# swasik/vector-store-text

Measured on AMD Instinct MI355X. Metric: kNN QPS @ recall@10>=0.95 (HNSW, 1000000 x 768 f32 cos), higher is better.
Workload: dtype f32

## Files before the change

### vector-store-text_amd/csrc/hnsw_regset.hpp

```cpp
#pragma once
#include <type_traits>

#include "hnsw_common.hpp"

namespace vsg {

#define VSG_KEY_EMPTY (~0ull)

#ifndef VSG_COMPACT_EARLY
#define VSG_COMPACT_EARLY 0
#endif

__device__ __forceinline__ uint64_t cand_key(float d, uint32_t id) {
    uint32_t b = __float_as_uint(d);
    if (b == 0x80000000u) b = 0u;
    const uint32_t u = (b & 0x80000000u) ? ~b : (b | 0x80000000u);
    return ((uint64_t)u << 32) | (id & VSG_ID_MASK);
}
__device__ __forceinline__ float key_dist(uint64_t k) {
    const uint32_t u = (uint32_t)(k >> 32);
    return __uint_as_float((u & 0x80000000u) ? (u & 0x7FFFFFFFu) : ~u);
}

__device__ __forceinline__ uint64_t shfl_xor64(uint64_t v, int o) {
    const uint32_t lo = (uint32_t)__shfl_xor((int)(uint32_t)v, o);
    const uint32_t hi = (uint32_t)__shfl_xor((int)(uint32_t)(v >> 32), o);
    return ((uint64_t)hi << 32) | lo;
}
__device__ __forceinline__ uint64_t readlane64(uint64_t v, int l) {
    const uint32_t lo = (uint32_t)__builtin_amdgcn_readlane((int)(uint32_t)v, l);
    const uint32_t hi = (uint32_t)__builtin_amdgcn_readlane((int)(uint32_t)(v >> 32), l);
    return ((uint64_t)hi << 32) | lo;
}
template <int CTRL> __device__ __forceinline__ uint64_t dpp64(uint64_t v) {
    const uint32_t lo = (uint32_t)__builtin_amdgcn_mov_dpp((int)(uint32_t)v, CTRL, 0xF, 0xF, false);
    const uint32_t hi = (uint32_t)__builtin_amdgcn_mov_dpp((int)(uint32_t)(v >> 32), CTRL, 0xF, 0xF, false);
    return ((uint64_t)hi << 32) | lo;
}
__device__ __forceinline__ uint64_t wave_min64(uint64_t v) {
#if VSG_DPP_REDUCE
    uint64_t w;
    w = dpp64<0xB1>(v);
    v = w < v ? w : v;
    w = dpp64<0x4E>(v);
    v = w < v ? w : v;
    w = dpp64<0x141>(v);
    v = w < v ? w : v;
    w = dpp64<0x140>(v);
    v = w < v ? w : v;
    const uint64_t r0 = readlane64(v, 0), r1 = readlane64(v, 16), r2 = readlane64(v, 32), r3 = readlane64(v, 48);
    const uint64_t a = r0 < r1 ? r0 : r1, b = r2 < r3 ? r2 : r3;
    return a < b ? a : b;
#else
#pragma unroll
    for (int o = 32; o > 0; o >>= 1) {
        const uint64_t w = shfl_xor64(v, o);
        v = w < v ? w : v;
    }
    return v;
#endif
}

template <int R> struct RegSet {
    uint64_t k[R];
    uint32_t expm;
    int size;
    uint64_t tkey;

    __device__ __forceinline__ void init(uint64_t first) {
#pragma unroll
        for (int r = 0; r < R; ++r) k[r] = VSG_KEY_EMPTY;
        if (lane_id() == 0) k[0] = first;
        expm = 0;
        size = 1;
        tkey = VSG_KEY_EMPTY;
    }

    __device__ __forceinline__ uint64_t min_unexpanded() const {
        uint64_t b = VSG_KEY_EMPTY;
#pragma unroll
        for (int r = 0; r < R; ++r)
            if (!((expm >> r) & 1u) && k[r] < b) b = k[r];
        return wave_min64(b);
    }

    __device__ __forceinline__ int count_below(uint64_t x) const {
        int c = 0;
#pragma unroll
        for (int r = 0; r < R; ++r) c += popc64(__ballot(k[r] < x));
        return c;
    }

    __device__ __forceinline__ void mark_expanded(uint64_t x) {
#pragma unroll
        for (int r = 0; r < R; ++r)
            if (k[r] == x) expm |= 1u << r;
    }

    __device__ __forceinline__ bool contains(uint64_t x) const {
        bool h = false;
#pragma unroll
        for (int r = 0; r < R; ++r) h = h || k[r] == x;
        return __ballot(h) != 0;
    }

    __device__ __forceinline__ void compact(int keep, uint32_t excl = 0) {
        uint32_t ph = 0;
        int need = keep;
#if VSG_COMPACT_EARLY
        int rsize = size;
        const int cap = keep + (64 * (R - 1) - keep) / 2;
#endif
#pragma unroll 1
        for (int b = 31; b >= 0; --b) {
            const uint32_t hm = b == 31 ? 0u : (~0u << (b + 1));
            int c = 0;
#pragma unroll
            for (int r = 0; r < R; ++r) {
                const uint32_t hi = (uint32_t)(k[r] >> 32);
                c += popc64(__ballot(k[r] != VSG_KEY_EMPTY && !((excl >> r) & 1u) && (hi & hm) == ph && !((hi >> b) & 1u)));
            }
            if (c < need) {
                need -= c;
                ph |= 1u << b;
#if VSG_COMPACT_EARLY
                rsize -= c;
#endif
            }
#if VSG_COMPACT_EARLY
            else {
                rsize = c;
            }
            const int kept = keep - need + rsize;
            if (b > 0 && kept <= cap) {
                const uint64_t cut = ((uint64_t)(ph | ((1u << b) - 1u)) << 32) | 0xFFFFFFFFull;
#pragma unroll
                for (int r = 0; r < R; ++r)
                    if (k[r] > cut) {
                        k[r] = VSG_KEY_EMPTY;
                        expm &= ~(1u << r);
                    }
                size = kept;
                tkey = cut;
                return;
            }
#endif
        }
        int ceq = 0;
#pragma unroll
        for (int r = 0; r < R; ++r)
            ceq += popc64(__ballot(k[r] != VSG_KEY_EMPTY && !((excl >> r) & 1u) && (uint32_t)(k[r] >> 32) == ph));
        uint64_t cut;
        if (need == ceq) {
            uint64_t mx = 0;
#pragma unroll
            for (int r = 0; r < R; ++r)
                if (k[r] != VSG_KEY_EMPTY && !((excl >> r) & 1u) && (uint32_t)(k[r] >> 32) == ph && k[r] > mx) mx = k[r];
#pragma unroll
            for (int o = 32; o > 0; o >>= 1) {
                const uint64_t w = shfl_xor64(mx, o);
                mx = w > mx ? w : mx;
            }
            cut = mx;
// ... 23 lines not shown
                expm &= ~(1u << r);
            }
        if (excl) {
            int c = 0;
#pragma unroll
            for (int r = 0; r < R; ++r) c += popc64(__ballot(k[r] != VSG_KEY_EMPTY));
            size = c;
        } else {
            size = keep;
        }
        tkey = cut;
    }

    __device__ __forceinline__ uint64_t bound_ef(int ef) const {
        uint32_t ph = 0;
        int need = ef;
#pragma unroll 1
        for (int b = 31; b >= 16; --b) {
            const uint32_t hm = b == 31 ? 0u : (~0u << (b + 1));
            int c = 0;
#pragma unroll
            for (int r = 0; r < R; ++r) {
                const uint32_t hi = (uint32_t)(k[r] >> 32);
                c += popc64(__ballot(k[r] != VSG_KEY_EMPTY && (hi & hm) == ph && !((hi >> b) & 1u)));
            }
            if (c < need) {
                need -= c;
                ph |= 1u << b;
            }
        }
        return ((uint64_t)(ph | 0xFFFFu) << 32) | 0xFFFFFFFFull;
    }

    __device__ __forceinline__ void fill(const uint64_t* sk, int nc) {
        int acc = 0;
#pragma unroll
        for (int r = 0; r < R; ++r) {
            if (acc < nc) {
                const bool fr = k[r] == VSG_KEY_EMPTY;
                const uint64_t em = __ballot(fr);
                const int idx = acc + lanes_below(em);
                if (fr && idx < nc) {
                    k[r] = sk[idx];
                    expm &= ~(1u << r);
                }
                acc += popc64(em);
            }
        }
        size += nc;
    }
};

template <int R>
__device__ __forceinline__ void admit(RegSet<R>& B, bool mine, uint64_t ck, bool lossy, int ef, uint64_t* sk,
                                      BeamProf* pf = nullptr) {
    (void)pf;
    const int lane = lane_id();
    bool valid = mine && ck < B.tkey;
    uint64_t vm = __ballot(valid);
    if (lossy && vm) {
        for (uint64_t mm = vm; mm; mm &= mm - 1) {
            const int j = __builtin_ctzll(mm);
            if (B.contains(readlane64(ck, j))) vm &= ~(1ull << j);
        }
        valid = (vm >> lane) & 1ull;
    }
    int nc = popc64(vm);
    if (nc && B.size + nc > 64 * R) {
#ifdef VSG_SEARCH_PROFILE
        const uint64_t tc = VSG_CYC();
#endif
        B.compact(ef);
        valid = valid && ck < B.tkey;
        vm = __ballot(valid);
        nc = popc64(vm);
#ifdef VSG_SEARCH_PROFILE
        if (pf) {
            pf->c_comp += VSG_CYC() - tc;
            pf->ncomp++;
        }
#endif
    }
    if (nc) {
        if (valid) sk[lanes_below(vm)] = ck;
        wave_sync();
        B.fill(sk, nc);
        wave_sync();
    }
}

struct NoSketch {};

template <int G, int VM, int U, typename T, int MET, int R, typename PRE = NoSketch>
__device__ __forceinline__ void beam_reg(const GraphDev& g, const QReg<G, VM, T>& q, int l, uint32_t ep, float dep, int ef, WaveLds& w,
                         RegSet<R>& B, uint64_t& ndist, uint64_t& nadj, BeamProf& pf, uint32_t self = VSG_EMPTY,
                         PRE* pre = nullptr) {
    const int lane = lane_id();
    [[maybe_unused]] int tau_size = -1;
    const int m0r = __builtin_amdgcn_readfirstlane(g.M0), mr = __builtin_amdgcn_readfirstlane(g.M);
    const int m = l == 0 ? m0r : mr;
    auto rfl_ptr = [](const uint32_t* p) {
        const uint64_t v = (uint64_t)p;
        const uint32_t lo = (uint32_t)__builtin_amdgcn_readfirstlane((int)(uint32_t)v);
        const uint32_t hi = (uint32_t)__builtin_amdgcn_readfirstlane((int)(uint32_t)(v >> 32));
        return (const uint32_t*)(((uint64_t)hi << 32) | lo);
    };
    const uint32_t* adj0 = rfl_ptr(g.adj0);
    const uint32_t* upper = rfl_ptr(g.upper);
    const uint32_t* upper_off = rfl_ptr(g.upper_off);
    w.vis.clear();
    if (ep != VSG_EMPTY) {
        if (lane == 0) {
            bool unrec;
            w.vis.insert(ep, unrec);
        }
        B.init(cand_key(dep, ep));
    } else {
        wave_sync();
#pragma unroll
        for (int r = 0; r < R; ++r)
            if (B.k[r] != VSG_KEY_EMPTY) {
                bool unrec;
                w.vis.insert((uint32_t)B.k[r] & VSG_ID_MASK, unrec);
            }
        B.expm = 0;
        B.tkey = VSG_KEY_EMPTY;
    }
    bool lossy = false;
    uint64_t* sk = reinterpret_cast<uint64_t*>(w.sd);
    wave_sync();
    auto row_of = [&](uint32_t n) {
        return l == 0 ? adj0 + (size_t)n * m0r : upper + ((size_t)upper_off[n] + (size_t)(l - 1)) * mr;
    };
    for (;;) {
        const uint64_t t0 = VSG_CLK();
        [[maybe_unused]] uint64_t c0c = VSG_CYC();
        const uint64_t a = B.min_unexpanded();
        if (a == VSG_KEY_EMPTY) break;
        if (B.size > ef && B.count_below(a) >= ef) break;
        B.mark_expanded(a);
        const uint32_t na = (uint32_t)a & VSG_ID_MASK;
        const uint32_t* row = row_of(na);
        ++nadj;
#ifdef VSG_SEARCH_PROFILE
        {
            const uint64_t c = VSG_CYC();
            pf.c_sel += c - c0c;
            pf.nexp++;
            c0c = c;
        }
#endif
        for (int c0 = 0; c0 < m; c0 += 64) {
            const uint32_t nb = c0 + lane < m ? row[c0 + lane] : VSG_EMPTY;
            const bool full = __ballot(nb != VSG_EMPTY) == ~0ull;
#ifdef VSG_SEARCH_PROFILE
            {
                const uint64_t c = VSG_CYC();
                pf.c_adj += c - c0c;
                c0c = c;
            }
#endif
            bool fresh = false, evicted = false;
            if (nb != VSG_EMPTY && nb != self) fresh = w.vis.insert(nb, evicted);
            const uint64_t mask = __ballot(fresh);
            lossy = lossy || __ballot(evicted) != 0;
            const int cnt0 = popc64(mask);
            if (fresh) w.todo[lanes_below(mask)] = nb;
            wave_sync();
            const uint64_t t1 = VSG_CLK();
            pf.adj += t1 - t0;
#ifdef VSG_SEARCH_PROFILE
            {
                const uint64_t c = VSG_CYC();
                pf.c_vis += c - c0c;
                c0c = c;
            }
#endif
            int cnt = cnt0;
            if constexpr (!std::is_same<PRE, NoSketch>::value) {
                if (cnt0) {
                    if (B.size >= ef && B.size != tau_size) {
                        const uint64_t tau = B.bound_ef(ef);
                        if (tau < B.tkey) B.tkey = tau;
                        tau_size = B.size;
                    }
                    if (B.tkey != VSG_KEY_EMPTY) cnt = pre->filter(w, cnt0, B.tkey);
                    pre->nexact += (uint32_t)cnt;
                }
            }
            ndist += (uint64_t)cnt0;
            if (cnt) {
#ifdef VSG_SEARCH_PROFILE
                rows_dist<G, VM, U, T, MET>(g.vecs, g.row_bytes, g.nchunks, w.todo, cnt, q, w.tdist, &pf.rows);
#else
                rows_dist<G, VM, U, T, MET>(g.vecs, g.row_bytes, g.nchunks, w.todo, cnt, q, w.tdist);
#endif
                wave_sync();
                const uint64_t ck = lane < cnt ? cand_key(w.tdist[lane], w.todo[lane]) : VSG_KEY_EMPTY;
                const uint64_t t2 = VSG_CLK();
                pf.dist += t2 - t1;
#ifdef VSG_SEARCH_PROFILE
                const uint64_t ca = VSG_CYC();
                admit<R>(B, lane < cnt, ck, lossy, ef, sk, &pf);
                c0c = VSG_CYC();
                pf.c_admit += c0c - ca;
#else
                admit<R>(B, lane < cnt, ck, lossy, ef, sk);
#endif
                pf.merge += VSG_CLK() - t2;
            }
            if (!full) break;
        }
    }
}


struct FiltState {
    uint32_t remm;
    int nlive;
    uint64_t maxlive;
    uint64_t rad0;
    uint32_t overflow;
    bool degraded;
};

__device__ __forceinline__ uint64_t wave_max64(uint64_t v) { return ~wave_min64(~v); }

template <int R> __device__ __forceinline__ int live_below(const RegSet<R>& B, const FiltState& F, uint64_t x) {
    int c = 0;
#pragma unroll
    for (int r = 0; r < R; ++r) c += popc64(__ballot(B.k[r] < x && !((F.remm >> r) & 1u)));
    return c;
}

template <int R> __device__ __forceinline__ void recount(RegSet<R>& B, FiltState& F) {
    int c = 0;
#pragma unroll
    for (int r = 0; r < R; ++r) {
        const bool e = B.k[r] == VSG_KEY_EMPTY;
        if (e) {
            F.remm &= ~(1u << r);
            B.expm &= ~(1u << r);
        }
        c += popc64(__ballot(!e));
    }
    B.size = c;
}

template <int R> __device__ __forceinline__ void compact_filt(RegSet<R>& B, FiltState& F, int ef) {
    if (F.nlive >= ef) {
        B.compact(ef, F.remm);
        F.nlive = ef;
        recount(B, F);
    }
}

template <int R>
__device__ __forceinline__ void fill_filt(RegSet<R>& B, FiltState& F, const uint64_t* sk, const uint32_t* sf, int nc) {
    int acc = 0;
#pragma unroll
    for (int r = 0; r < R; ++r) {
        if (acc < nc) {
            const bool fr = B.k[r] == VSG_KEY_EMPTY;
            const uint64_t em = __ballot(fr);
            const int idx = acc + lanes_below(em);
            if (fr && idx < nc) {
                B.k[r] = sk[idx];
                B.expm &= ~(1u << r);
                if (sf[idx]) F.remm |= 1u << r;
                else F.remm &= ~(1u << r);
            }
            acc += popc64(em);
        }
    }
    B.size += nc;
}

template <int R>
__device__ __forceinline__ void admit_filt(RegSet<R>& B, FiltState& F, bool mine, uint64_t ck, bool rem, bool lossy,
                                           int ef, uint64_t* sk, uint32_t* sf) {
    const int lane = lane_id();
    bool valid = mine && ck < B.tkey && !(F.degraded && rem);
    uint64_t vm = __ballot(valid);
    if (lossy && vm) {
        for (uint64_t mm = vm; mm; mm &= mm - 1) {
            const int j = __builtin_ctzll(mm);
            if (B.contains(readlane64(ck, j))) vm &= ~(1ull << j);
        }
        valid = (vm >> lane) & 1ull;
    }
    int nc = popc64(vm);
    if (nc && B.size + nc > 64 * R) {
        compact_filt(B, F, ef);
        valid = valid && ck < B.tkey;
        vm = __ballot(valid);
        nc = popc64(vm);
        if (B.size + nc > 64 * R) {
            const uint64_t before = (uint64_t)B.size;
#pragma unroll
            for (int r = 0; r < R; ++r)
                if ((F.remm >> r) & 1u) B.k[r] = VSG_KEY_EMPTY;
            recount(B, F);
            F.overflow += (uint32_t)(before - (uint64_t)B.size) + (uint32_t)popc64(__ballot(valid && rem));
            F.degraded = true;
            valid = valid && !rem;
            vm = __ballot(valid);
// ... 143 lines not shown
```

### vector-store-text_amd/csrc/hnsw_search_reg.hip

```cpp
#include <hip/hip_runtime.h>

#include <map>
#include <type_traits>
#include <mutex>
#include <tuple>

#include "hnsw_common.hpp"
#include "hnsw_regset.hpp"
#include "sketch_device.hpp"
#include "vsg_dispatch.hpp"

namespace vsg {

#ifndef VSG_SEARCH_ATTR
#define VSG_SEARCH_ATTR
#endif
template <int G, int VM, int U, typename T, int MET, int R, bool PF>
__device__ __forceinline__ void search_reg_one(const SearchParams& p, int qi, uint8_t* smem) {
    const int lane = lane_id();
    const GraphDev g = to_dev(p.g);
    WaveLds w = carve(smem, 0, p.hash_size, 0);
    uint64_t ndist = 0, nadj = 0;
    BeamProf pf;
    [[maybe_unused]] const uint64_t cq0 = VSG_CYC(), tq0 = VSG_CLK();
    int count = 0;
    uint64_t* ok = p.out_keys + (size_t)qi * p.k;
    float* od = p.out_dist + (size_t)qi * p.k;
    if (p.entry != VSG_EMPTY) {
        QReg<G, VM, T> q;
        q.load(p.queries + (size_t)qi * g.row_bytes, g.nchunks);
        uint32_t cur = p.entry;
        float dcur = dist_one<G, VM, U, T, MET>(g, q, cur, w);
        ++ndist;
        RegSet<R> B;
        using SS = SketchShape<G, VM>;
        using Pre = std::conditional_t<PF, SketchPre<SS::GS, SS::VMS, SS::US>, NoSketch>;
        Pre pre_s;
        Pre* pre = nullptr;
        if constexpr (PF) {
            pre_s.sk = p.sk;
            pre_s.meta = reinterpret_cast<const float2*>(p.sk_meta);
            pre_s.stride = p.sk_stride;
            pre_s.schunks = (int)(p.sk_stride / 16);
            pre_s.q.stage(p.queries + (size_t)qi * g.row_bytes, g.nchunks, p.sk_dim,
                          smem + wave_lds_bytes(p.hash_size, 0, 0));
            pre = &pre_s;
        }
        if (p.upper_ef > 1 && p.max_level >= 1) {
#ifdef VSG_UPPER_ALL_LEVELS
            beam_reg<G, VM, U, T, MET, R>(g, q, p.max_level, cur, dcur, min(p.upper_ef, p.ef), w, B, ndist, nadj, pf);
            for (int l = p.max_level - 1; l >= 1; --l)
                beam_reg<G, VM, U, T, MET, R>(g, q, l, VSG_EMPTY, 0.f, min(p.upper_ef, p.ef), w, B, ndist, nadj, pf);
#else
            for (int l = p.max_level; l >= 2; --l) greedy_level<G, VM, U, T, MET>(g, q, l, cur, dcur, w, ndist, nadj);
            beam_reg<G, VM, U, T, MET, R>(g, q, 1, cur, dcur, min(p.upper_ef, p.ef), w, B, ndist, nadj, pf);
#endif
            beam_reg<G, VM, U, T, MET, R, Pre>(g, q, 0, VSG_EMPTY, 0.f, p.ef, w, B, ndist, nadj, pf, VSG_EMPTY, pre);
        } else {
            [[maybe_unused]] const uint64_t cd0 = VSG_CYC();
            for (int l = p.max_level; l >= 1; --l) greedy_level<G, VM, U, T, MET>(g, q, l, cur, dcur, w, ndist, nadj);
#ifdef VSG_SEARCH_PROFILE
            pf.c_desc += VSG_CYC() - cd0;
#endif
            beam_reg<G, VM, U, T, MET, R, Pre>(g, q, 0, cur, dcur, p.ef, w, B, ndist, nadj, pf, VSG_EMPTY, pre);
        }
        if constexpr (PF) {
            if (lane == 0 && p.stats) {
                atomicAdd(&p.stats[18], (unsigned long long)pre_s.nsketch);
                atomicAdd(&p.stats[19], (unsigned long long)pre_s.nexact);
            }
        }
        uint32_t alive = 0;
#pragma unroll
        for (int r = 0; r < R; ++r)
            if (B.k[r] != VSG_KEY_EMPTY && !(p.flags[(uint32_t)B.k[r] & VSG_ID_MASK] & 1)) alive |= 1u << r;
        uint32_t* sel = w.vis.tab;
        const int lim = min(p.ef, B.size);
        for (int x = 0; x < lim && count < p.k; ++x) {
            uint64_t b = VSG_KEY_EMPTY;
#pragma unroll
            for (int r = 0; r < R; ++r) b = B.k[r] < b ? B.k[r] : b;
            b = wave_min64(b);
            if (b == VSG_KEY_EMPTY) break;
            bool live = false;
#pragma unroll
            for (int r = 0; r < R; ++r)
                if (B.k[r] == b) {
                    live = (alive >> r) & 1u;
                    B.k[r] = VSG_KEY_EMPTY;
                }
            if (__ballot(live)) {
                if (lane == 0) {
                    od[count] = key_dist(b);
                    sel[count] = (uint32_t)b & VSG_ID_MASK;
                }
                ++count;
            }
        }
        wave_sync();
        for (int j = lane; j < count; j += 64) ok[j] = p.keys ? p.keys[sel[j]] : (uint64_t)sel[j];
    }
    for (int j = count + lane; j < p.k; j += 64) {
        ok[j] = ~0ull;
        od[j] = __builtin_inff();
    }
    if (lane == 0) {
        if (p.out_counts) p.out_counts[qi] = (uint32_t)count;
        if (p.stats) {
            atomicAdd(&p.stats[0], (unsigned long long)ndist);
            atomicAdd(&p.stats[1], (unsigned long long)nadj);
            atomicAdd(&p.stats[2], 1ull);
#ifdef VSG_SEARCH_PROFILE
            atomicAdd(&p.stats[10], (unsigned long long)pf.adj);
            atomicAdd(&p.stats[11], (unsigned long long)pf.dist);
            atomicAdd(&p.stats[12], (unsigned long long)pf.merge);
            atomicAdd(&p.stats[20], (unsigned long long)pf.c_sel);
            atomicAdd(&p.stats[21], (unsigned long long)pf.c_adj);
            atomicAdd(&p.stats[22], (unsigned long long)pf.c_vis);
            atomicAdd(&p.stats[23], (unsigned long long)pf.rows.wait);
            atomicAdd(&p.stats[24], (unsigned long long)pf.rows.valu);
            atomicAdd(&p.stats[25], (unsigned long long)pf.c_admit);
            atomicAdd(&p.stats[26], (unsigned long long)pf.c_comp);
            atomicAdd(&p.stats[27], (unsigned long long)pf.c_desc);
            atomicAdd(&p.stats[28], (unsigned long long)pf.nexp | ((unsigned long long)pf.ncomp << 40));
            atomicAdd(&p.stats[29], (unsigned long long)pf.rows.passes);
            atomicAdd(&p.stats[30], (unsigned long long)(VSG_CYC() - cq0));
            atomicAdd(&p.stats[31], (unsigned long long)(VSG_CLK() - tq0));
#endif
        }
    }
}

template <int G, int VM> constexpr bool persist_shape() { return G * VM * 16 >= 1024; }

template <int G, int VM, int U, typename T, int MET, int R, bool PF = false>
__global__ __launch_bounds__(64) VSG_SEARCH_ATTR void hnsw_search_reg_kernel(SearchParams p) {
    extern __shared__ __attribute__((aligned(16))) uint8_t smem[];
    if constexpr (persist_shape<G, VM>()) {
        if (p.qnext) {
            for (;;) {
                int qi = 0;
                if (lane_id() == 0) qi = (int)atomicAdd(p.qnext, 1u);
                qi = __builtin_amdgcn_readfirstlane(qi);
                if (qi >= p.nq) break;
                search_reg_one<G, VM, U, T, MET, R, PF>(p, qi, smem);
                wave_sync();
            }
            return;
        }
    }
    int qi = blockIdx.x;
    if (p.xcd_map) {
        const int nq = p.nq, qd = nq >> 3, rm = nq & 7;
        const int x = blockIdx.x & 7, j = blockIdx.x >> 3;
        qi = x * qd + min(x, rm) + j;
    }
    search_reg_one<G, VM, U, T, MET, R, PF>(p, qi, smem);
}

template <int G, int VM, typename T, int MET, int R> constexpr bool prefilter_shape() {
    return std::is_same<T, float>::value && MET == MET_DOT && G * VM * 16 >= 1024 && G * VM <= 512 && R <= 8;
}

static inline int reg_rows(int ef) { return ef <= 64 ? 2 : ef <= 192 ? 4 : ef <= 448 ? 8 : 17; }

bool search_prefilter_supported(Storage st, MetricKind mk, int nchunks, int ef) {
    return st == ST_F32 && mk == MK_DOT && nchunks * 16 >= 1024 && nchunks <= 512 && ef >= 1 && ef <= 448;
}

size_t search_reg_lds_bytes(int hash) { return wave_lds_bytes(hash, 0, 0); }

static double env_frac(const char* name, double dflt) {
    const char* e = getenv(name);
    return e ? atof(e) : dflt;
}

static int resident_blocks(const void* kern, size_t lds) {
    static std::mutex mu;
    static std::map<std::tuple<int, const void*, size_t>, int> cache;
    int dev = 0;
    (void)hipGetDevice(&dev);
    std::lock_guard<std::mutex> lk(mu);
    auto it = cache.find({dev, kern, lds});
    if (it != cache.end()) return it->second;
    int cus = 0, per_cu = 0;
    (void)hipDeviceGetAttribute(&cus, hipDeviceAttributeMultiprocessorCount, dev);
    (void)hipOccupancyMaxActiveBlocksPerMultiprocessor(&per_cu, kern, 64, lds);
    const int r = std::max(1, per_cu * cus);
    cache[{dev, kern, lds}] = r;
    return r;
}

hipError_t launch_search_reg(Storage st, MetricKind mk, const SearchParams& p, hipStream_t s) {
    if (p.nq <= 0) return hipSuccess;
    if (p.ef < 1 || p.ef > 1024 || p.k > p.ef || p.hash_size < p.k) return hipErrorInvalidValue;
    const size_t lds_plain = search_reg_lds_bytes(p.hash_size);
    hipError_t err = hipSuccess;
    int rows = reg_rows(p.ef);
    if (const char* e = getenv("VSG_SEARCH_REG_ROWS")) {
        const int r = atoi(e);
        if ((r == 2 || r == 4 || r == 8 || r == 17) && 64 * r >= p.ef + 64) rows = r;
    }
    auto launch_rows = [&](auto rtag) {
        constexpr int R = decltype(rtag)::value;
        auto body = [&](auto sh, auto tt, auto mt) {
            constexpr int G = decltype(sh)::G, VM = decltype(sh)::VM, U = decltype(sh)::U;
            using T = typename decltype(tt)::T;
            constexpr int MET = decltype(mt)::MET;
            auto run = [&](auto kern, size_t lds) {
                if (lds > 65536)
                    (void)hipFuncSetAttribute((const void*)kern, hipFuncAttributeMaxDynamicSharedMemorySize, (int)lds);
                constexpr int CH = 1 << 22;
                for (int off = 0; off < p.nq && err == hipSuccess; off += CH) {
                    SearchParams c = p;
                    c.nq = min(CH, p.nq - off);
                    c.queries = p.queries + (size_t)off * p.g.row_bytes;
                    c.out_keys = p.out_keys + (size_t)off * p.k;
                    c.out_dist = p.out_dist + (size_t)off * p.k;
                    c.out_counts = p.out_counts ? p.out_counts + off : nullptr;
                    unsigned grid = (unsigned)c.nq;
                    if (persist_shape<G, VM>() && p.qnext) {
                        static const double frac = std::min(1.0, std::max(0.05, env_frac("VSG_SEARCH_PERSIST_FRAC", 0.75)));
                        const int res = std::max(1, (int)(frac * resident_blocks((const void*)kern, lds)));
                        grid = (unsigned)std::max(1, std::min(c.nq, res));
                        err = hipMemsetAsync(p.qnext, 0, sizeof(unsigned), s);
                        if (err != hipSuccess) break;
                    }
                    hipLaunchKernelGGL(kern, dim3(grid), dim3(64), lds, s, c);
                    err = hipGetLastError();
                }
            };
            if constexpr (prefilter_shape<G, VM, T, MET, R>()) {
                if (p.sk) {
                    run(hnsw_search_reg_kernel<G, VM, U, T, MET, R, true>, lds_plain + SketchShape<G, VM>::LDS_BYTES);
                    return;
                }
            }
            run(hnsw_search_reg_kernel<G, VM, U, T, MET, R>, lds_plain);
        };
        if constexpr (R == 17) dispatch_all<SHAPE_GENERIC>(st, mk, p.g.nchunks, body);
        else if constexpr (R == 2) dispatch_all<SHAPE_SEARCH_SMALL_EF>(st, mk, p.g.nchunks, body);
        else dispatch_all<SHAPE_SEARCH>(st, mk, p.g.nchunks, body);
    };
    if (rows == 2) launch_rows(std::integral_constant<int, 2>{});
    else if (rows == 4) launch_rows(std::integral_constant<int, 4>{});
    else if (rows == 8) launch_rows(std::integral_constant<int, 8>{});
    else launch_rows(std::integral_constant<int, 17>{});
    return err;
}

}
```

### vector-store-text_amd/csrc/sketch.hpp

```cpp
#pragma once
#include <math.h>
#include <stdint.h>

#if defined(__HIPCC__) || defined(__CUDACC__)
#define VSG_HD __host__ __device__
#else
#define VSG_HD
#endif

namespace vsg {

struct SketchMeta {
    float scale;
    float err;
};

static inline VSG_HD size_t sketch_stride(int dim) { return ((size_t)dim + 127) / 128 * 128; }

static inline VSG_HD float sketch_maxabs(const float* x, int dim) {
    float m = 0.f;
    for (int i = 0; i < dim; ++i) {
        const float a = fabsf(x[i]);
        if (!(a <= 3.4028234e38f)) return INFINITY;
        m = a > m ? a : m;
    }
    return m;
}

static inline VSG_HD float sketch_scale(float maxabs) {
    if (!(maxabs >= 1e-30f) || !(maxabs <= 1e30f)) return 0.f;
    return maxabs / 127.f;
}

static inline VSG_HD uint8_t sketch_quant(float x, float scale) {
    float k = rintf(x / scale);
    k = k > 127.f ? 127.f : (k < -127.f ? -127.f : k);
    return (uint8_t)((int)k + 128);
}

static inline VSG_HD float sketch_res2(float x, float scale, uint8_t u) {
    const float r = fmaf(-scale, (float)((int)u - 128), x);
    return r * r;
}

static inline VSG_HD float sketch_err(float sum_res2, float sum_x2, float scale, int dim) {
    if (!(scale > 0.f)) return INFINITY;
    const float u = 5.9604645e-8f;
    const float infl = 1.f + (float)(dim + 8) * 2.f * u;
    const float e = sqrtf(sum_res2) * infl;
    const float xn = sqrtf(sum_x2) * infl;
    const float sd = sqrtf((float)dim) * 1.0001f;
    const float mag = xn + 2.f * e;
    const float slack = (float)(dim + 8) * u * 1.01f * (384.f * sd * scale + mag) + 4.f * u * mag;
    const float r = (e + slack) * (1.f + 8.f * u);
    return r == r ? r : INFINITY;
}

static inline VSG_HD SketchMeta sketch_row(const float* x, int dim, uint8_t* out) {
    const size_t stride = sketch_stride(dim);
    SketchMeta m;
    m.scale = sketch_scale(sketch_maxabs(x, dim));
    if (!(m.scale > 0.f)) {
        for (size_t i = 0; i < stride; ++i) out[i] = 128;
        m.scale = 0.f;
        m.err = INFINITY;
        return m;
    }
    float r2 = 0.f, x2 = 0.f;
    for (int i = 0; i < dim; ++i) {
        out[i] = sketch_quant(x[i], m.scale);
        r2 += sketch_res2(x[i], m.scale, out[i]);
        x2 = fmaf(x[i], x[i], x2);
    }
    for (size_t i = (size_t)dim; i < stride; ++i) out[i] = 128;
    m.err = sketch_err(r2, x2, m.scale, dim);
    if (!(m.err < INFINITY)) m.scale = 0.f;
    return m;
}

static inline VSG_HD float sketch_qnorm_up(float sum_q2, int dim) {
    return sqrtf(sum_q2) * (1.f + (float)(dim + 8) * 1.1920929e-7f);
}

}
```

### vector-store-text_amd/csrc/sketch_device.hpp

```cpp
#pragma once
#include "hnsw_common.hpp"
#include "hnsw_regset.hpp"

namespace vsg {

template <int G, int VM> struct SketchShape {
    static constexpr int SC = G * VM / 4;
    static constexpr int GS = SC <= 48 ? 16 : SC <= 128 ? 32 : 64;
    static constexpr int VMS = (SC + GS - 1) / GS;
    static constexpr int US = VMS <= 1 ? 8 : VMS <= 3 ? 4 : 2;
    static constexpr int LDS_BYTES = VMS * 4 * GS * 16;
};

template <int GS, int VMS> struct SketchQ {
    static constexpr int UNITS = VMS * 4 * GS;
    const uint4* img;
    float sumq, qn;

    __device__ __forceinline__ void stage(const uint8_t* __restrict__ qrow, int nchunks, int dim, uint8_t* lds) {
        uint4* dst = reinterpret_cast<uint4*>(lds);
        float s = 0.f, s2 = 0.f;
        for (int t = lane_id(); t < UNITS; t += 64) {
            const int v = t / (4 * GS), j = (t / GS) % 4, sl = t % GS;
            const int fc = (v * GS + sl) * 4 + j;
            uint4 raw = make_uint4(0u, 0u, 0u, 0u);
            if (fc < nchunks) raw = *reinterpret_cast<const uint4*>(qrow + (size_t)fc * 16);
            dst[t] = raw;
            const float e[4] = {__uint_as_float(raw.x), __uint_as_float(raw.y), __uint_as_float(raw.z),
                                __uint_as_float(raw.w)};
#pragma unroll
            for (int i = 0; i < 4; ++i) {
                s += e[i];
                s2 = __builtin_fmaf(e[i], e[i], s2);
            }
        }
#pragma unroll
        for (int o = 32; o > 0; o >>= 1) {
            s += __shfl_xor(s, o);
            s2 += __shfl_xor(s2, o);
        }
        img = dst;
        sumq = s;
        qn = __builtin_sqrtf(s2) * (1.f + (float)(dim + 8) * 1.1920929e-7f);
        wave_sync();
    }
};

template <int GS, int VMS, int US>
__device__ __forceinline__ void rows_sketch(const uint8_t* __restrict__ sk, size_t stride, int schunks,
                                            const float2* __restrict__ meta, const uint32_t* ids, int count,
                                            const SketchQ<GS, VMS>& q, float* out) {
    constexpr int RS = 64 / GS;
    const int lane = lane_id();
    const int sub = lane / GS;
    const int sl = lane % GS;
    for (int base = 0; base < count; base += RS * US) {
        uint4 raw[US][VMS];
        float2 mt[US];
#pragma unroll
        for (int u = 0; u < US; ++u) {
            const int r = base + u * RS + sub;
            const uint32_t id = ids[r < count ? r : count - 1];
            const uint8_t* row = sk + (size_t)id * stride;
            mt[u] = meta[id];
#pragma unroll
            for (int v = 0; v < VMS; ++v) {
                const int c = v * GS + sl;
                raw[u][v] = *reinterpret_cast<const uint4*>(row + (size_t)(c < schunks ? c : schunks - 1) * 16);
            }
        }
        uint4 qx[VMS][4];
#pragma unroll
        for (int v = 0; v < VMS; ++v) {
#pragma unroll
            for (int j = 0; j < 4; ++j) qx[v][j] = q.img[(v * 4 + j) * GS + sl];
        }
#pragma unroll
        for (int u = 0; u < US; ++u) {
            if (base + u * RS >= count) break;
            float acc = 0.f;
#pragma unroll
            for (int v = 0; v < VMS; ++v) {
                const uint32_t w[4] = {raw[u][v].x, raw[u][v].y, raw[u][v].z, raw[u][v].w};
#pragma unroll
                for (int j = 0; j < 4; ++j) {
                    acc = __builtin_fmaf((float)(w[j] & 0xFFu), __uint_as_float(qx[v][j].x), acc);
                    acc = __builtin_fmaf((float)((w[j] >> 8) & 0xFFu), __uint_as_float(qx[v][j].y), acc);
                    acc = __builtin_fmaf((float)((w[j] >> 16) & 0xFFu), __uint_as_float(qx[v][j].z), acc);
                    acc = __builtin_fmaf((float)(w[j] >> 24), __uint_as_float(qx[v][j].w), acc);
                }
            }
            acc = group_sum0<GS>(acc);
            const int r = base + u * RS + sub;
            if (sl == 0 && r < count) {
                const float t = acc - 128.f * q.sumq;
                out[r] = __builtin_fmaf(q.qn, mt[u].y, mt[u].x * t);
            }
        }
    }
}

template <int GS, int VMS, int US> struct SketchPre {
    const uint8_t* sk;
    const float2* meta;
    size_t stride;
    int schunks;
    SketchQ<GS, VMS> q;
    uint32_t nsketch = 0, nexact = 0;

    __device__ __forceinline__ int filter(WaveLds& w, int cnt, uint64_t tkey) {
        const int lane = lane_id();
        rows_sketch<GS, VMS, US>(sk, stride, schunks, meta, w.todo, cnt, q, w.tdist);
        wave_sync();
        nsketch += (uint32_t)cnt;
        const float ub = lane < cnt ? w.tdist[lane] : 0.f;
        const uint32_t cid = lane < cnt ? w.todo[lane] : 0u;
        const bool finite = __builtin_fabsf(ub) < __builtin_inff();
        const bool keep = lane < cnt && !(finite && cand_key(1.f - ub, 0u) >= tkey);
        const uint64_t km = __ballot(keep);
        wave_sync();
        if (keep) w.todo[lanes_below(km)] = cid;
        wave_sync();
        return popc64(km);
    }
};

}
```

### vector-store-text_amd/csrc/vsg_index.cpp

```cpp
#include <hip/hip_runtime.h>

#include <algorithm>
#include <atomic>
#include <chrono>
#include <cmath>
#include <cstddef>
#include <cstdio>
#include <cstdlib>
#include <cstring>
#include <deque>
#include <mutex>
#include <shared_mutex>
#include <string>
#include <system_error>
#include <thread>
#include <unordered_set>
#include <vector>

#include "../../include/vsg.h"
#include "keymap.hpp"
#include "roctx_range.hpp"
#include "search_plan.hpp"
#include "sketch.hpp"
#include "vsg_kernels.hpp"
// ... 1653 lines not shown
            for (; j < n; ++j) {
                const uint64_t k = keys[j];
                if (k >= KeyMap::DEAD || seen.count(k)) break;
                uint32_t slot = 0;
                const bool live = h->keys.find(k, &slot);
                const size_t av = avail + (live && slot != h->entry ? 1 : 0);
                const int kd = reuse && av > 0 ? 1 : 0;
                if (kind < 0) {
                    kind = kd;
                    C = batch ? batch : std::max<size_t>(1, h->live / (kd ? div : 8));
                } else if (kd != kind || j - i >= C) {
                    break;
                }
                avail = av - (size_t)kd;
                seen.insert(k);
                if (live) rm.push_back(k);
            }
        }
        if (hold && j == n && j - i < C) {
            for (size_t t = i; status && t < n; ++t) status[t] = VSG_HELD;
            break;
        }
        int rc = rm.empty() ? VSG_OK : remove_locked(h, rm.data(), rm.size(), nullptr);
        if (rc == VSG_OK)
            rc = add_locked(h, keys + i, vecs + i * (size_t)h->dim, j - i, device_src, user_stream, j - i);
        record(i, j, rc);
        i = j;
    }
    if (n_applied) *n_applied = i;
    if (first) g_last_error = first_msg;
    return first;
}

int vsg_index_replace(vsg_index_t* h, const uint64_t* keys, const float* vectors, size_t n, size_t batch,
                      uint32_t flags, int* status, size_t* n_applied) {
    VSG_RANGE();
    return replace_common(h, keys, vectors, n, batch, flags, status, n_applied, false, nullptr);
}

int vsg_index_replace_device(vsg_index_t* h, const uint64_t* keys, const float* vectors_device, size_t n,
                             size_t batch, int* status, void* stream) {
    VSG_RANGE();
    return replace_common(h, keys, vectors_device, n, batch, 0, status, nullptr, true, (hipStream_t)stream);
}

constexpr size_t WS_MAX = 4;

static bool same_stream(hipStream_t a, hipStream_t b) { return a == b && a != nullptr && a != hipStreamPerThread; }

static int ws_acquire(vsg_index* h, size_t bytes, hipStream_t s, Workspace** out) {
    Workspace* w = nullptr;
    {
        std::lock_guard<std::mutex> lk(h->ctx_mu);
        const size_t none = h->ws_free.size();
        size_t ready = none, fit = none, big = none;
        for (size_t i = 0; i < none; ++i) {
            Workspace* c = h->ws_free[i];
            if (c->pending && !same_stream(c->last, s) && hipEventQuery(c->done) == hipSuccess) c->pending = false;
            const bool nowait = !c->pending || same_stream(c->last, s);
            if (c->cap >= bytes && nowait && (ready == none || c->cap < h->ws_free[ready]->cap)) ready = i;
            if (c->cap >= bytes && (fit == none || c->cap < h->ws_free[fit]->cap)) fit = i;
            if (big == none || c->cap > h->ws_free[big]->cap) big = i;
        }
        size_t best = ready;
        if (best == none && h->ws_count >= WS_MAX) best = fit != none ? fit : big;
        if (best < none) {
            w = h->ws_free[best];
            h->ws_free.erase(h->ws_free.begin() + (long)best);
        } else {
            ++h->ws_count;
        }
    }
    auto drop = [&](Workspace* d) {
        delete d;
        std::lock_guard<std::mutex> lk(h->ctx_mu);
        --h->ws_count;
    };
    if (!w) {
        w = new Workspace;
        w->home = h->stream;
        if (hipEventCreateWithFlags(&w->done, hipEventDisableTiming) != hipSuccess) {
            drop(w);
            return fail(VSG_EDEVICE, "hipEventCreate failed");
        }
    }
    if (w->cap < bytes) {
        if (w->pending) (void)hipEventSynchronize(w->done);
        w->pending = false;
        dev_free(w->base, h->stream);
        w->base = nullptr;
        const size_t want = std::max(bytes, w->cap * 2);
        w->cap = 0;
        if (pool_alloc((void**)&w->base, want, s) != hipSuccess) {
            drop(w);
            return fail(VSG_ENOMEM, "search workspace");
        }
        w->cap = want;
    } else if (w->pending && !same_stream(w->last, s)) {
        const hipError_t e = hipStreamWaitEvent(s, w->done, 0);
        if (e != hipSuccess) {
            std::lock_guard<std::mutex> lk(h->ctx_mu);
            h->ws_free.push_back(w);
            return fail(VSG_EDEVICE, std::string("hipStreamWaitEvent: ") + hipGetErrorString(e));
        }
    }
    *out = w;
    return VSG_OK;
}

static void ws_release(vsg_index* h, Workspace* w, hipStream_t s) {
    w->pending = hipEventRecord(w->done, s) == hipSuccess;
    w->last = s;
    if (!w->pending) (void)hipStreamSynchronize(s);
    std::lock_guard<std::mutex> lk(h->ctx_mu);
    h->ws_free.push_back(w);
}

#define ROW_TRY(expr)                                          \
    do {                                                       \
        if (hipError_t e__ = (expr)) return step = #expr, e__; \
    } while (0)
static int row_copy_fail(const char* step, hipError_t e) {
    return fail(VSG_EDEVICE, std::string(step) + ": " + hipGetErrorString(e));
}

static int ensure_shadow(vsg_index* h, hipStream_t s) {
    RowCopy& c = h->shadow;
    std::lock_guard<std::mutex> g(c.mu);
    const char* step = "hipStreamSynchronize(s)";
    const hipError_t e = row_copy_ensure(
        h, c, h->cap, h->pub_slots, s,
        [&](size_t, hipStream_t s) {
            row_copy_drop(h, c, s, h->d_vecs16);
            ROW_TRY(dev_alloc(&h->d_vecs16, h->cap * h->row_bytes16, s));
            return hipSuccess;
        },
        [&](size_t slots, hipStream_t s) {
            if (h->shadow.cap > slots)
                ROW_TRY(hipMemsetAsync(h->d_vecs16 + slots * h->row_bytes16, 0, (h->shadow.cap - slots) * h->row_bytes16, s));
            return hipSuccess;
        },
        [&](size_t, size_t slots, hipStream_t s) {
            ROW_TRY(launch_shadow_f16(h->d_vecs, h->row_bytes, h->shadow.rows, slots, h->dim, h->d_vecs16,
                                      h->row_bytes16, s));
            return hipSuccess;
        });
    return e == hipSuccess ? VSG_OK : row_copy_fail(step, e);
}

static bool prefilter_on(const vsg_index* h, size_t ef, size_t nq) {
    if (h->f16_trav || !search_prefilter_supported(h->st, h->mk, h->nchunks, (int)ef)) return false;
    if (h->prefilter >= 0) return h->prefilter != 0;
    if (const char* e = getenv("VSG_SEARCH_PREFILTER")) return atof(e) != 0;
    return ef <= 64 && nq >= 4096;
}

static bool ensure_sketch(vsg_index* h, hipStream_t s) {
    RowCopy& c = h->sketch;
    std::lock_guard<std::mutex> g(c.mu);
    if (env_double("VSG_TEST_FAIL_SKETCH", 0) != 0) return false;
    const hipError_t e = row_copy_ensure(
        h, c, h->cap, h->pub_slots, s,
        [&](size_t cap, hipStream_t s) {
            row_copy_drop(h, c, s, h->d_sketch, h->d_sketch_meta);
            hipError_t a = dev_alloc(&h->d_sketch, cap * sketch_stride(h->dim), s);
            if (a == hipSuccess) a = dev_alloc(&h->d_sketch_meta, cap * 2, s);
            if (a != hipSuccess) {
                (void)hipGetLastError();
                row_copy_drop(h, c, s, h->d_sketch, h->d_sketch_meta);
            }
            return a;
        },
        [&](size_t, hipStream_t s) { return hipMemsetAsync(h->d_sketch_meta, 0xFF, c.cap * 2 * sizeof(float), s); },
        [&](size_t first, size_t last, hipStream_t s) {
            return launch_sketch_rows(h->d_vecs, h->row_bytes, first, last, h->dim, h->d_sketch, h->d_sketch_meta, s);
        });
    if (e != hipSuccess) c.gen = ~0ull;
    return e == hipSuccess;
}

static bool ktile_on(const vsg_index* h) {
    return (h->opt.flags & VSG_FLAG_EXACT_ONLY) && h->st == ST_F32 && (h->row_bytes / 4) % 32 == 0 &&
           env_double("VSG_EXACT_KTILE", 1) != 0;
}

static int ensure_ktile(vsg_index* h, size_t slots, hipStream_t s) {
    RowCopy& c = h->ktile;
    std::lock_guard<std::mutex> g(c.mu);
    if (env_double("VSG_TEST_FAIL_KTILE", 0) != 0) return fail(VSG_ENOMEM, "K-tiled copy (injected failure)");
    const char* step = "hipStreamSynchronize(s)";
    const hipError_t e = row_copy_ensure(
        h, c, (h->cap + KTILE_ROWS - 1) / KTILE_ROWS * KTILE_ROWS, slots, s,
        [&](size_t want_cap, hipStream_t s) {
            row_copy_drop(h, c, s, h->d_ktile);
            ROW_TRY(dev_alloc(&h->d_ktile, want_cap * (h->row_bytes / 4), s));
            ROW_TRY(hipMemsetAsync(h->d_ktile, 0, want_cap * h->row_bytes, s));
            return hipSuccess;
        },
        [](size_t, hipStream_t) { return hipSuccess; },
        [&](size_t, size_t slots, hipStream_t s) {
            ROW_TRY(launch_ktile_rows(reinterpret_cast<const float*>(h->d_vecs), (int)(h->row_bytes / 4), h->ktile.rows,
                                      slots, h->d_ktile, s));
            return hipSuccess;
        });
    return e == hipSuccess ? VSG_OK : row_copy_fail(step, e);
}
#undef ROW_TRY

static_assert(PLAN_MFMA_BQ == MFMA_BQ && PLAN_MFMA_BR == MFMA_BR, "search_plan.hpp plans the tile the MFMA kernel runs");

extern "C++" struct SearchCall {
    const float* q_dev;
    size_t nq, k;
    uint64_t* ok;
    float* od;
    uint32_t* oc;
    hipStream_t s;
    uint8_t* base;
    SearchLayout at;
    template <typename X>
    X* region(size_t off) const {
        return reinterpret_cast<X*>(base + off);
    }
};

static int search_launch_rc(hipError_t err) {
    if (err != hipSuccess) return fail(VSG_EDEVICE, std::string("search launch: ") + hipGetErrorString(err));
    return VSG_OK;
}

static hipError_t merge_parts_two_stage(float* pd, uint32_t* pi, const ExactPlan& plan, size_t nq, size_t k, int kin,
                                        const uint64_t* keys, uint64_t* ok, float* od, uint32_t* oc, hipStream_t s) {
    const int ng = plan.ngroups;
    if (ng) {
        MergeParams g1{};
        g1.part_d = pd;
        g1.part_i = pi;
        g1.nq = (int)(nq * ng);
        g1.parts = 64;
        g1.k = (int)k;
        g1.kin = kin;
        g1.out_part_d = pd + plan.np_lists;
        g1.out_part_i = pi + plan.np_lists;
        const hipError_t err = launch_merge_parts(g1, s);
        if (err != hipSuccess) return err;
    }
    MergeParams mp{};
    mp.part_d = ng ? pd + plan.np_lists : pd;
    mp.part_i = ng ? pi + plan.np_lists : pi;
    mp.nq = (int)nq;
    mp.parts = ng ? ng : plan.lists();
    mp.k = (int)k;
    mp.kin = ng ? 0 : kin;
    mp.keys = keys;
    mp.out_keys = ok;
    mp.out_dist = od;
    mp.out_counts = oc;
    return launch_merge_parts(mp, s);
}

static int run_exact_mfma(vsg_index* h, const SearchCall& c, const ExactPlan& plan, size_t slots) {
    float* pd = c.region<float>(c.at.part_d);
    uint32_t* pi = c.region<uint32_t>(c.at.part_i);
    MfmaExactParams mp{};
    mp.vecs = reinterpret_cast<const float*>(h->d_vecs);
    if (ktile_on(h)) {
        const int rk = ensure_ktile(h, slots, c.s);
        if (rk) return rk;
        mp.ktile = h->d_ktile;
    }
    mp.sqnorm = h->d_sqnorm;
    mp.queries = c.region<const float>(c.at.queries);
    mp.qsqnorm = c.region<const float>(c.at.qnorms);
    mp.row_floats = (int)(h->row_bytes / 4);
    mp.nq = (int)c.nq;
    mp.nslots = slots;
    mp.flags = h->d_flags;
    mp.qtiles = plan.qtiles;
    mp.splits = (int)plan.splits;
    mp.tiles_per_split = (int)plan.tiles_per_split;
    mp.kmax = plan.kmax;
    mp.bq = plan.bq;
    mp.br = plan.br;
    mp.part_d = pd;
    mp.part_i = pi;
    hipError_t err = launch_mfma_exact(h->mk, mp, c.s);
    if (err == hipSuccess)
        err = merge_parts_two_stage(pd, pi, plan, c.nq, c.k, plan.kmax, h->d_keys, c.ok, c.od, c.oc, c.s);
    return search_launch_rc(err);
}

static int run_exact_valu(vsg_index* h, const SearchCall& c, const ExactPlan& plan, size_t slots) {
    float* pd = c.region<float>(c.at.part_d);
    uint32_t* pi = c.region<uint32_t>(c.at.part_i);
    ExactParams ep{};
    ep.vecs = h->d_vecs;
    ep.row_bytes = h->row_bytes;
    ep.nchunks = h->nchunks;
    ep.queries = c.region<const uint8_t>(c.at.queries);
    ep.nq = (int)c.nq;
    ep.k = (int)c.k;
    ep.nslots = slots;
    ep.rows_per_block = std::max(plan.rows_per_block, 1);
    ep.nblocks = plan.nblocks;
    ep.flags = h->d_flags;
    ep.part_d = pd;
    ep.part_i = pi;
// ... 1024 lines not shown
```

Measured before the change: 4.153 million.

## Quantize sketch query to int16 hi/lo and use sdot4 for prefilter bounds

The sketch prefilter now quantizes the query into two signed 8-bit planes (hi/lo of an int16) and computes the bound with integer sdot4 instead of float FMAs over unpacked bytes. This halves the query LDS image and cuts ALU work. The change also tightens the pruning threshold early from the ef-th bound, uses a separate persistent-grid fraction for prefilter kernels, adjusts the unroll shape, and enables the prefilter for ef up to 192 at large batch sizes. The added quantization-error term in the bound keeps it conservative but loosens it slightly, which could reduce pruning.

```diff
diff --git a/vector-store-text_amd/csrc/hnsw_regset.hpp b/vector-store-text_amd/csrc/hnsw_regset.hpp
--- a/vector-store-text_amd/csrc/hnsw_regset.hpp
+++ b/vector-store-text_amd/csrc/hnsw_regset.hpp
@@ -9,6 +9,9 @@
 
 #ifndef VSG_COMPACT_EARLY
 #define VSG_COMPACT_EARLY 0
+#endif
+#ifndef VSG_TAU_EARLY
+#define VSG_TAU_EARLY 1
 #endif
 
 __device__ __forceinline__ uint64_t cand_key(float d, uint32_t id) {
@@ -338,6 +341,13 @@
 #endif
         for (int c0 = 0; c0 < m; c0 += 64) {
             const uint32_t nb = c0 + lane < m ? row[c0 + lane] : VSG_EMPTY;
+            if constexpr (!std::is_same<PRE, NoSketch>::value) {
+                if (VSG_TAU_EARLY && c0 == 0 && B.size >= ef && B.size != tau_size) {
+                    const uint64_t tau = B.bound_ef(ef);
+                    if (tau < B.tkey) B.tkey = tau;
+                    tau_size = B.size;
+                }
+            }
             const bool full = __ballot(nb != VSG_EMPTY) == ~0ull;
 #ifdef VSG_SEARCH_PROFILE
             {
diff --git a/vector-store-text_amd/csrc/hnsw_search_reg.hip b/vector-store-text_amd/csrc/hnsw_search_reg.hip
--- a/vector-store-text_amd/csrc/hnsw_search_reg.hip
+++ b/vector-store-text_amd/csrc/hnsw_search_reg.hip
@@ -33,7 +33,7 @@
         float dcur = dist_one<G, VM, U, T, MET>(g, q, cur, w);
         ++ndist;
         RegSet<R> B;
-        using SS = SketchShape<G, VM>;
+        using SS = SketchShape<G, VM, U>;
         using Pre = std::conditional_t<PF, SketchPre<SS::GS, SS::VMS, SS::US>, NoSketch>;
         Pre pre_s;
         Pre* pre = nullptr;
@@ -170,6 +170,10 @@
 
 size_t search_reg_lds_bytes(int hash) { return wave_lds_bytes(hash, 0, 0); }
 
+#ifndef VSG_PERSIST_FRAC_PF
+#define VSG_PERSIST_FRAC_PF 1.0
+#endif
+
 static double env_frac(const char* name, double dflt) {
     const char* e = getenv(name);
     return e ? atof(e) : dflt;
@@ -207,7 +211,7 @@
             constexpr int G = decltype(sh)::G, VM = decltype(sh)::VM, U = decltype(sh)::U;
             using T = typename decltype(tt)::T;
             constexpr int MET = decltype(mt)::MET;
-            auto run = [&](auto kern, size_t lds) {
+            auto run = [&](auto kern, size_t lds, bool pf = false) {
                 if (lds > 65536)
                     (void)hipFuncSetAttribute((const void*)kern, hipFuncAttributeMaxDynamicSharedMemorySize, (int)lds);
                 constexpr int CH = 1 << 22;
@@ -221,7 +225,9 @@
                     unsigned grid = (unsigned)c.nq;
                     if (persist_shape<G, VM>() && p.qnext) {
                         static const double frac = std::min(1.0, std::max(0.05, env_frac("VSG_SEARCH_PERSIST_FRAC", 0.75)));
-                        const int res = std::max(1, (int)(frac * resident_blocks((const void*)kern, lds)));
+                        static const double frac_pf =
+                            std::min(1.0, std::max(0.05, env_frac("VSG_SEARCH_PERSIST_FRAC", VSG_PERSIST_FRAC_PF)));
+                        const int res = std::max(1, (int)((pf ? frac_pf : frac) * resident_blocks((const void*)kern, lds)));
                         grid = (unsigned)std::max(1, std::min(c.nq, res));
                         err = hipMemsetAsync(p.qnext, 0, sizeof(unsigned), s);
                         if (err != hipSuccess) break;
@@ -232,7 +238,9 @@
             };
             if constexpr (prefilter_shape<G, VM, T, MET, R>()) {
                 if (p.sk) {
-                    run(hnsw_search_reg_kernel<G, VM, U, T, MET, R, true>, lds_plain + SketchShape<G, VM>::LDS_BYTES);
+                    constexpr int UP = prefilter_u<G, VM, U>();
+                    run(hnsw_search_reg_kernel<G, VM, UP, T, MET, R, true>, lds_plain + SketchShape<G, VM, UP>::LDS_BYTES,
+                        true);
                     return;
                 }
             }
diff --git a/vector-store-text_amd/csrc/sketch.hpp b/vector-store-text_amd/csrc/sketch.hpp
--- a/vector-store-text_amd/csrc/sketch.hpp
+++ b/vector-store-text_amd/csrc/sketch.hpp
@@ -82,4 +82,47 @@
     return sqrtf(sum_q2) * (1.f + (float)(dim + 8) * 1.1920929e-7f);
 }
 
+
+static inline VSG_HD float sketch_qscale(float maxabs) {
+    if (!(maxabs >= 9.094947e-13f) || !(maxabs <= 1.0995116e12f)) return 0.f;
+    return maxabs / 32512.f;
 }
+
+static inline VSG_HD int sketch_q16(float q, float sq) {
+    float k = rintf(q / sq);
+    k = k > 32512.f ? 32512.f : (k < -32512.f ? -32512.f : k);
+    return (int)k;
+}
+static inline VSG_HD int sketch_q16_hi(int q16) { return (q16 + 32768 + 128) / 256 - 128; }
+static inline VSG_HD int sketch_q16_lo(int q16) { return q16 - 256 * sketch_q16_hi(q16); }
+
+static inline VSG_HD float sketch_qres2(float q, float sq, int q16) {
+    const float r = fmaf(-sq, (float)q16, q);
+    return r * r;
+}
+
+struct SketchQuery {
+    float sq, qe, qn;
+};
+
+static inline VSG_HD SketchQuery sketch_query(float maxabs, float sum_res2, float sum_q2, int dim) {
+    SketchQuery r;
+    r.sq = sketch_qscale(maxabs);
+    r.qn = sketch_qnorm_up(sum_q2, dim);
+    const float infl = 1.f + (float)(dim + 8) * 1.1920929e-7f;
+    const float qerr = sqrtf(sum_res2) * infl + 9.094947e-13f * maxabs;
+    r.qe = qerr * (127.f * sqrtf((float)dim)) * 1.001f;
+    if (!(r.qe < INFINITY) || !(r.qn < INFINITY)) r.sq = 0.f;
+    return r;
+}
+
+#define VSG_SKETCH_PMIN 8.2718061e-25f
+
+static inline VSG_HD float sketch_upper(const SketchQuery& q, SketchMeta m, int H, int L) {
+    const float p = q.sq * m.scale;
+    const float S = fmaf(256.f, (float)H, (float)L);
+    const float ub = fmaf(p, S, fmaf(q.qe, m.scale, q.qn * m.err));
+    return p >= VSG_SKETCH_PMIN ? ub : INFINITY;
+}
+
+}
diff --git a/vector-store-text_amd/csrc/sketch_device.hpp b/vector-store-text_amd/csrc/sketch_device.hpp
--- a/vector-store-text_amd/csrc/sketch_device.hpp
+++ b/vector-store-text_amd/csrc/sketch_device.hpp
@@ -1,47 +1,99 @@
 #pragma once
 #include "hnsw_common.hpp"
 #include "hnsw_regset.hpp"
+#include "sketch.hpp"
 
 namespace vsg {
 
-template <int G, int VM> struct SketchShape {
+template <int G, int VM, int U> struct SketchShape {
     static constexpr int SC = G * VM / 4;
     static constexpr int GS = SC <= 48 ? 16 : SC <= 128 ? 32 : 64;
     static constexpr int VMS = (SC + GS - 1) / GS;
-    static constexpr int US = VMS <= 1 ? 8 : VMS <= 3 ? 4 : 2;
-    static constexpr int LDS_BYTES = VMS * 4 * GS * 16;
+    static constexpr int US = VMS <= 1 ? 8 : VMS <= 3 ? (U >= 4 ? 4 : 2) : 2;
+    static constexpr int LDS_BYTES = VMS * 2 * GS * 16;
 };
 
+#ifndef VSG_PREFILTER_U2
+#define VSG_PREFILTER_U2 0
+#endif
+template <int G, int VM, int U> constexpr int prefilter_u() { return VSG_PREFILTER_U2 && VM == 6 && U > 2 ? 2 : U; }
+
+template <int G> __device__ __forceinline__ int group_isum0(int a) {
+    if constexpr (G >= 64) a += __shfl_xor(a, 32);
+    if constexpr (G >= 32) a += __builtin_amdgcn_ds_swizzle(a, 0x401F);
+    if constexpr (G >= 16) a += __builtin_amdgcn_mov_dpp(a, 0x108, 0xF, 0xF, true);
+    if constexpr (G >= 8) a += __builtin_amdgcn_mov_dpp(a, 0x104, 0xF, 0xF, true);
+    if constexpr (G >= 4) a += __builtin_amdgcn_mov_dpp(a, 0x4E, 0xF, 0xF, true);
+    if constexpr (G >= 2) a += __builtin_amdgcn_mov_dpp(a, 0xB1, 0xF, 0xF, true);
+    return a;
+}
+
 template <int GS, int VMS> struct SketchQ {
-    static constexpr int UNITS = VMS * 4 * GS;
+    static constexpr int CHUNKS = VMS * GS;
     const uint4* img;
-    float sumq, qn;
+    SketchQuery k;
+
+    static __device__ __forceinline__ void elems(const uint8_t* __restrict__ qrow, int nchunks, int c, float (&e)[16]) {
+#pragma unroll
+        for (int j = 0; j < 4; ++j) {
+            const int fc = c * 4 + j;
+            uint4 raw = make_uint4(0u, 0u, 0u, 0u);
+            if (fc < nchunks) raw = *reinterpret_cast<const uint4*>(qrow + (size_t)fc * 16);
+            e[j * 4 + 0] = __uint_as_float(raw.x);
+            e[j * 4 + 1] = __uint_as_float(raw.y);
+            e[j * 4 + 2] = __uint_as_float(raw.z);
+            e[j * 4 + 3] = __uint_as_float(raw.w);
+        }
+    }
 
     __device__ __forceinline__ void stage(const uint8_t* __restrict__ qrow, int nchunks, int dim, uint8_t* lds) {
         uint4* dst = reinterpret_cast<uint4*>(lds);
-        float s = 0.f, s2 = 0.f;
-        for (int t = lane_id(); t < UNITS; t += 64) {
-            const int v = t / (4 * GS), j = (t / GS) % 4, sl = t % GS;
-            const int fc = (v * GS + sl) * 4 + j;
-            uint4 raw = make_uint4(0u, 0u, 0u, 0u);
-            if (fc < nchunks) raw = *reinterpret_cast<const uint4*>(qrow + (size_t)fc * 16);
-            dst[t] = raw;
-            const float e[4] = {__uint_as_float(raw.x), __uint_as_float(raw.y), __uint_as_float(raw.z),
-                                __uint_as_float(raw.w)};
+        img = dst;
+        float mx = 0.f, s2 = 0.f;
+        for (int c = lane_id(); c < CHUNKS; c += 64) {
+            float e[16];
+            elems(qrow, nchunks, c, e);
 #pragma unroll
-            for (int i = 0; i < 4; ++i) {
-                s += e[i];
+            for (int i = 0; i < 16; ++i) {
+                const float a = __builtin_fabsf(e[i]);
+                if (!(a <= 3.4028234e38f)) mx = __builtin_inff();
+                mx = a > mx ? a : mx;
                 s2 = __builtin_fmaf(e[i], e[i], s2);
             }
         }
 #pragma unroll
         for (int o = 32; o > 0; o >>= 1) {
-            s += __shfl_xor(s, o);
+            const float m2 = __shfl_xor(mx, o);
+            mx = m2 > mx ? m2 : mx;
             s2 += __shfl_xor(s2, o);
         }
-        img = dst;
-        sumq = s;
-        qn = __builtin_sqrtf(s2) * (1.f + (float)(dim + 8) * 1.1920929e-7f);
+        const float sq = sketch_qscale(mx);
+        float r2 = 0.f;
+        if (sq > 0.f) {
+            for (int c = lane_id(); c < CHUNKS; c += 64) {
+                float e[16];
+                elems(qrow, nchunks, c, e);
+                uint32_t hw[4], lw[4];
+#pragma unroll
+                for (int j = 0; j < 4; ++j) {
+                    hw[j] = 0u;
+                    lw[j] = 0u;
+#pragma unroll
+                    for (int i = 0; i < 4; ++i) {
+                        const int q16 = sketch_q16(e[j * 4 + i], sq);
+                        r2 += sketch_qres2(e[j * 4 + i], sq, q16);
+                        hw[j] |= ((uint32_t)sketch_q16_hi(q16) & 0xFFu) << (8 * i);
+                        lw[j] |= ((uint32_t)sketch_q16_lo(q16) & 0xFFu) << (8 * i);
+                    }
+                }
+                const int v = c / GS, sl = c % GS;
+                dst[(v * 2 + 0) * GS + sl] = make_uint4(hw[0], hw[1], hw[2], hw[3]);
+                dst[(v * 2 + 1) * GS + sl] = make_uint4(lw[0], lw[1], lw[2], lw[3]);
+            }
+#pragma unroll
+            for (int o = 32; o > 0; o >>= 1) r2 += __shfl_xor(r2, o);
+        }
+        k = sketch_query(mx, r2, s2, dim);
         wave_sync();
     }
 };
@@ -69,33 +121,32 @@
                 raw[u][v] = *reinterpret_cast<const uint4*>(row + (size_t)(c < schunks ? c : schunks - 1) * 16);
             }
         }
-        uint4 qx[VMS][4];
+        uint4 qh[VMS], ql[VMS];
 #pragma unroll
         for (int v = 0; v < VMS; ++v) {
-#pragma unroll
-            for (int j = 0; j < 4; ++j) qx[v][j] = q.img[(v * 4 + j) * GS + sl];
+            qh[v] = q.img[(v * 2 + 0) * GS + sl];
+            ql[v] = q.img[(v * 2 + 1) * GS + sl];
         }
 #pragma unroll
         for (int u = 0; u < US; ++u) {
             if (base + u * RS >= count) break;
-            float acc = 0.f;
+            int ah = 0, al = 0;
 #pragma unroll
             for (int v = 0; v < VMS; ++v) {
                 const uint32_t w[4] = {raw[u][v].x, raw[u][v].y, raw[u][v].z, raw[u][v].w};
+                const uint32_t h[4] = {qh[v].x, qh[v].y, qh[v].z, qh[v].w};
+                const uint32_t l[4] = {ql[v].x, ql[v].y, ql[v].z, ql[v].w};
 #pragma unroll
                 for (int j = 0; j < 4; ++j) {
-                    acc = __builtin_fmaf((float)(w[j] & 0xFFu), __uint_as_float(qx[v][j].x), acc);
-                    acc = __builtin_fmaf((float)((w[j] >> 8) & 0xFFu), __uint_as_float(qx[v][j].y), acc);
-                    acc = __builtin_fmaf((float)((w[j] >> 16) & 0xFFu), __uint_as_float(qx[v][j].z), acc);
-                    acc = __builtin_fmaf((float)(w[j] >> 24), __uint_as_float(qx[v][j].w), acc);
+                    const int x = (int)(w[j] ^ 0x80808080u);
+                    ah = __builtin_amdgcn_sdot4(x, (int)h[j], ah, false);
+                    al = __builtin_amdgcn_sdot4(x, (int)l[j], al, false);
                 }
             }
-            acc = group_sum0<GS>(acc);
+            ah = group_isum0<GS>(ah);
+            al = group_isum0<GS>(al);
             const int r = base + u * RS + sub;
-            if (sl == 0 && r < count) {
-                const float t = acc - 128.f * q.sumq;
-                out[r] = __builtin_fmaf(q.qn, mt[u].y, mt[u].x * t);
-            }
+            if (sl == 0 && r < count) out[r] = sketch_upper(q.k, SketchMeta{mt[u].x, mt[u].y}, ah, al);
         }
     }
 }
@@ -109,6 +160,7 @@
     uint32_t nsketch = 0, nexact = 0;
 
     __device__ __forceinline__ int filter(WaveLds& w, int cnt, uint64_t tkey) {
+        if (!(q.k.sq > 0.f)) return cnt;
         const int lane = lane_id();
         rows_sketch<GS, VMS, US>(sk, stride, schunks, meta, w.todo, cnt, q, w.tdist);
         wave_sync();
diff --git a/vector-store-text_amd/csrc/vsg_index.cpp b/vector-store-text_amd/csrc/vsg_index.cpp
--- a/vector-store-text_amd/csrc/vsg_index.cpp
+++ b/vector-store-text_amd/csrc/vsg_index.cpp
@@ -1829,7 +1829,7 @@
     if (h->f16_trav || !search_prefilter_supported(h->st, h->mk, h->nchunks, (int)ef)) return false;
     if (h->prefilter >= 0) return h->prefilter != 0;
     if (const char* e = getenv("VSG_SEARCH_PREFILTER")) return atof(e) != 0;
-    return ef <= 64 && nq >= 4096;
+    return (ef <= 64 && nq >= 4096) || (ef <= 192 && nq >= 10000);
 }
 
 static bool ensure_sketch(vsg_index* h, hipStream_t s) {
```

After: 4.779 million (median of 6 runs). 15.1% higher.
